# rrwick/Filtlong

Measured on AMD Instinct MI355X. Metric: Mbases/s scored+sorted, higher is better.
Workload: dtype f64; 1 GPU; 10,000,000 synthetic reads per GPU x gamma(k=4) mean 10 kbp, Phred-only, --target_bases 50008889515 (50% of bases); C2; reads_total=10000000, bases_total=100017779031, window_size=250, parallelism=1 GPU, device=AMD Radeon Graphics (gfx950:sramecc+:xnack-), gpus_visible=1, cut=select

## Files before the change

### filtlong_amd/csrc/fold_map.h

```cpp
#pragma once

#include <hip/hip_runtime.h>

namespace flx_fold {

constexpr int NO_MAP = -2147483647 - 1;

__device__ __forceinline__ int exponent_of(double v) {
    return (int)((__double_as_longlong(v) >> 52) & 0x7ff) - 1023;
}

struct Map2 {
    long long a0, a1;
};
__device__ __forceinline__ Map2 compose(const Map2 &a, const Map2 &b) {
    Map2 c;
    c.a0 = a.a0 + ((a.a0 & 1) ? b.a1 : b.a0);
    c.a1 = a.a1 + (((1 + a.a1) & 1) ? b.a1 : b.a0);
    return c;
}

__device__ __forceinline__ Map2 elem_map(double v, int e, bool &ok) {
    Map2 m;
    m.a0 = m.a1 = 0;
    const unsigned long long bits = (unsigned long long)__double_as_longlong(v);
    if ((bits << 1) == 0) return m;
    const int eb = (int)((bits >> 52) & 0x7ff);
    unsigned long long mx = bits & 0x000fffffffffffffull;
    int ex;
    if (eb == 0) ex = -1022;
    else { mx |= 1ull << 52; ex = eb - 1023; }
    const int sh = e - ex;
    if (sh < 0) { ok = false; return m; }
    if (sh == 0) { m.a0 = m.a1 = (long long)mx; return m; }
    if (sh >= 55) return m;
    const unsigned long long f = mx >> sh;
    const unsigned long long rem = mx & ((1ull << sh) - 1ull);
    const unsigned long long half = 1ull << (sh - 1);
    if (rem > half) m.a0 = m.a1 = (long long)(f + 1);
    else if (rem < half) m.a0 = m.a1 = (long long)f;
    else {
        m.a0 = (long long)(f + (f & 1));
        m.a1 = (long long)(f + ((f + 1) & 1));
    }
    return m;
}

__device__ __forceinline__ double readlane_f64(double v, int src) {
    const long long b = __double_as_longlong(v);
    const int lo = __builtin_amdgcn_readlane((int)(b & 0xffffffffll), src);
    const int hi = __builtin_amdgcn_readlane((int)(b >> 32), src);
    return __longlong_as_double(((long long)hi << 32) | (unsigned int)lo);
}

__device__ __forceinline__ bool normal_positive(double S) {
    const unsigned long long sb = (unsigned long long)__double_as_longlong(S);
    const int eb = (int)((sb >> 52) & 0x7ff);
    return (sb >> 63) == 0 && eb >= 1 && eb <= 2046;
}

}
```

### filtlong_amd/csrc/stats.hip

```cpp
#include <cmath>

#include "flx_internal.h"
#include "rank_internal.h"
#include "fold_map.h"

using namespace flx_fold;

namespace {

constexpr int CHUNK = 512;
constexpr int PER_LANE = CHUNK / 64;

struct Identity {
    double mean;
    __device__ __forceinline__ double operator()(double x) const { return x; }
};
struct SqDev {
    const double *mean;
    __device__ __forceinline__ double operator()(double x) const {
        const double d = x - *mean;
        return d * d;
    }
};

struct ChunkMeta {
    long long a0, a1;
    int e;
    int pad;
};

template <typename F>
__global__ void __launch_bounds__(256) k_chunk_sums(uint64_t n, const double *x, F f, double *chunk_sum, double *chunk_start,
                                                    unsigned char *chunk_clean, double *minmax) {
    const int lane = threadIdx.x & 63;
    const uint64_t chunk = (uint64_t)blockIdx.x * 4 + (threadIdx.x >> 6);
    const uint64_t base = chunk * CHUNK;
    if (base >= n) return;
    double acc = 0.0;
    bool clean = true;
    double lo = 100.0, hi = 0.0;
#pragma unroll
    for (int k = 0; k < PER_LANE; ++k) {
        const uint64_t i = base + (uint64_t)k * 64 + lane;
        if (i < n) {
            const double raw = x[i];
            const double v = f(raw);
            acc += v;
            clean = clean && (v >= 0.0) && (v < __longlong_as_double(0x7ff0000000000000ll));
            if (raw > hi) hi = raw;
            if (raw < lo) lo = raw;
        }
    }
    for (int o = 32; o > 0; o >>= 1) {
        acc += __shfl_xor(acc, o, 64);
        const double h2 = __shfl_xor(hi, o, 64), l2 = __shfl_xor(lo, o, 64);
        if (h2 > hi) hi = h2;
        if (l2 < lo) lo = l2;
    }
    const bool all_clean = __all(clean);
    if (lane == 0) {
        chunk_sum[chunk] = acc;
        chunk_start[chunk] = acc;
        chunk_clean[chunk] = all_clean ? 1 : 0;
        if (minmax) {
            minmax[2 * chunk] = lo;
            minmax[2 * chunk + 1] = hi;
        }
    }
}

__global__ void __launch_bounds__(256) k_minmax(uint64_t n_chunks, const double *minmax, double *out) {
    double lo = 100.0, hi = 0.0;
    for (uint64_t c = threadIdx.x; c < n_chunks; c += 256) {
        const double l = minmax[2 * c], h = minmax[2 * c + 1];
        if (l < lo) lo = l;
        if (h > hi) hi = h;
    }
    for (int o = 32; o > 0; o >>= 1) {
        const double l2 = __shfl_xor(lo, o, 64), h2 = __shfl_xor(hi, o, 64);
        if (l2 < lo) lo = l2;
        if (h2 > hi) hi = h2;
    }
    __shared__ double sl[4], sh[4];
    if ((threadIdx.x & 63) == 0) {
        sl[threadIdx.x >> 6] = lo;
        sh[threadIdx.x >> 6] = hi;
    }
    __syncthreads();
    if (threadIdx.x == 0) {
        for (int i = 1; i < 4; ++i) {
            if (sl[i] < lo) lo = sl[i];
            if (sh[i] > hi) hi = sh[i];
        }
        out[0] = lo;
        out[1] = hi;
    }
}

template <typename F>
__global__ void __launch_bounds__(256) k_chunk_maps(uint64_t n, const double *x, F f, const double *chunk_start,
                                                    const double *chunk_sum, const unsigned char *chunk_clean,
                                                    ChunkMeta *meta) {
    const int lane = threadIdx.x & 63;
    const uint64_t chunk = (uint64_t)blockIdx.x * 4 + (threadIdx.x >> 6);
    const uint64_t base = chunk * CHUNK;
    if (base >= n) return;
    const double p0 = chunk_start[chunk] * (1.0 - 1e-9);
    const double p1 = (chunk_start[chunk] + chunk_sum[chunk]) * (1.0 + 1e-9);
    int e = NO_MAP;
    if (chunk_clean[chunk] && p0 > 2.3e-308 && p1 < 1e300 && exponent_of(p0) == exponent_of(p1)) e = exponent_of(p0);
    Map2 m;
    m.a0 = m.a1 = 0;
    bool ok = true;
    if (e != NO_MAP) {
#pragma unroll
        for (int k = 0; k < PER_LANE; ++k) {
            const uint64_t i = base + (uint64_t)lane * PER_LANE + k;
            if (i < n) m = compose(m, elem_map(f(x[i]), e, ok));
        }
#pragma unroll
        for (int o = 1; o < 64; o <<= 1) {
            Map2 nb;
            nb.a0 = __shfl_down(m.a0, o, 64);
            nb.a1 = __shfl_down(m.a1, o, 64);
            if ((lane & (2 * o - 1)) == 0) m = compose(m, nb);
        }
        if (!__all(ok)) e = NO_MAP;
    }
    if (lane == 0) {
        ChunkMeta cm;
        cm.a0 = m.a0;
        cm.a1 = m.a1;
        cm.e = e;
        cm.pad = 0;
        meta[chunk] = cm;
    }
}

__global__ void __launch_bounds__(256) k_batch_maps(const ChunkMeta *meta, uint64_t n_chunks, ChunkMeta *batch) {
    const int lane = threadIdx.x & 63;
    const uint64_t b = (uint64_t)blockIdx.x * 4 + (threadIdx.x >> 6);
    const uint64_t c0 = b * 64;
    if (c0 >= n_chunks) return;
    ChunkMeta mine;
    mine.a0 = mine.a1 = 0;
    mine.e = NO_MAP;
    if (c0 + lane < n_chunks) mine = meta[c0 + lane];
    const int e0 = __builtin_amdgcn_readfirstlane(mine.e);
    const bool full = c0 + 64 <= n_chunks;
    Map2 m;
    m.a0 = mine.a0;
    m.a1 = mine.a1;
    const bool ok = full && e0 != NO_MAP && __all(mine.e == e0);
    if (ok) {
#pragma unroll
        for (int o = 1; o < 64; o <<= 1) {
            Map2 nb;
            nb.a0 = __shfl_down(m.a0, o, 64);
            nb.a1 = __shfl_down(m.a1, o, 64);
            if ((lane & (2 * o - 1)) == 0) m = compose(m, nb);
        }
    }
    if (lane == 0) {
        ChunkMeta out;
        out.a0 = m.a0;
        out.a1 = m.a1;
        out.e = ok ? e0 : NO_MAP;
        out.pad = 0;
        batch[b] = out;
    }
}

__device__ __forceinline__ bool apply_map(double &S, int e, long long a0, long long a1) {
    const unsigned long long sb = (unsigned long long)__double_as_longlong(S);
    const int se = (int)((sb >> 52) & 0x7ff) - 1023;
    if (se != e || (sb >> 63) != 0 || a0 < 0 || a1 < 0) return false;
    const unsigned long long m = (sb & 0x000fffffffffffffull) | (1ull << 52);
    const unsigned long long m2 = m + (unsigned long long)((m & 1) ? a1 : a0);
    if (m2 > (1ull << 53)) return false;
    if (m2 == (1ull << 53)) S = __longlong_as_double((long long)(((unsigned long long)(e + 1 + 1023)) << 52));
    else S = __longlong_as_double((long long)((((unsigned long long)(e + 1023)) << 52) | (m2 & 0x000fffffffffffffull)));
    return true;
}

__device__ __forceinline__ Map2 wave_scan_maps(Map2 m, int lane) {
#pragma unroll
    for (int o = 1; o < 64; o <<= 1) {
        Map2 prev;
        prev.a0 = __shfl_up(m.a0, o, 64);
        prev.a1 = __shfl_up(m.a1, o, 64);
        if (lane >= o) m = compose(prev, m);
    }
    return m;
}

__device__ __forceinline__ int wave_apply_prefix(double &S, int e, Map2 m, bool usable, int start, int lane) {
    const bool good = usable && m.a0 >= 0 && m.a1 >= 0;
    const unsigned long long bad = __ballot(lane >= start && !good);
    const int first_bad = bad ? (int)__ffsll((long long)bad) - 1 : 64;
    if (lane < start || lane >= first_bad) m.a0 = m.a1 = 0;
    const Map2 P = wave_scan_maps(m, lane);
    const unsigned long long sb = (unsigned long long)__double_as_longlong(S);
    const unsigned long long ms = (sb & 0x000fffffffffffffull) | (1ull << 52);
    const unsigned long long m2 = ms + (unsigned long long)((ms & 1) ? P.a1 : P.a0);
    const bool inside = m2 <= (1ull << 53);
    const unsigned long long out = __ballot(lane >= start && lane < first_bad && !inside);
    const int f = out ? (int)__ffsll((long long)out) - 1 : first_bad;
    if (f > start) {
        const unsigned int lo = (unsigned int)__builtin_amdgcn_readlane((int)(m2 & 0xffffffffull), f - 1);
        const unsigned int hi = (unsigned int)__builtin_amdgcn_readlane((int)(m2 >> 32), f - 1);
        const unsigned long long r = ((unsigned long long)hi << 32) | lo;
        if (r == (1ull << 53)) S = __longlong_as_double((long long)(((unsigned long long)(e + 1 + 1023)) << 52));
        else S = __longlong_as_double((long long)((((unsigned long long)(e + 1023)) << 52) | (r & 0x000fffffffffffffull)));
    }
    return f;
}

template <typename F>
__global__ void __launch_bounds__(64) k_walk(uint64_t n, const double *x, F f, const ChunkMeta *meta, const ChunkMeta *batch,
                                             uint64_t n_chunks, flx_stats_dev *out, int second) {
    const int lane = threadIdx.x;
    double S = 0.0;
    unsigned long long n_serial = 0;
    const uint64_t n_batches = (n_chunks + 63) / 64;
    for (uint64_t bb = 0; bb < n_batches && S == S; bb += 64) {
        ChunkMeta bm;
        bm.a0 = bm.a1 = 0;
        bm.e = NO_MAP;
        if (bb + lane < n_batches) bm = batch[bb + lane];
        const int bcnt = (int)((n_batches - bb) < 64 ? (n_batches - bb) : 64);
        int bs = 0;
        while (bs < bcnt && S == S) {
            int fb = bs;
            if (normal_positive(S)) {
                const int e = exponent_of(S);
                Map2 m;
                m.a0 = bm.a0;
                m.a1 = bm.a1;
                fb = wave_apply_prefix(S, e, m, lane < bcnt && bm.e == e, bs, lane);
            }
            if (fb >= bcnt) break;
            const uint64_t cb = (bb + fb) * 64;
            ChunkMeta mine;
            mine.a0 = mine.a1 = 0;
            mine.e = NO_MAP;
            if (cb + lane < n_chunks) mine = meta[cb + lane];
            const int cnt = (int)((n_chunks - cb) < 64 ? (n_chunks - cb) : 64);
            int cs = 0;
            while (cs < cnt && S == S) {
                int fc = cs;
                if (normal_positive(S)) {
                    const int e = exponent_of(S);
                    Map2 m;
                    m.a0 = mine.a0;
                    m.a1 = mine.a1;
                    fc = wave_apply_prefix(S, e, m, lane < cnt && mine.e == e, cs, lane);
                }
                if (fc >= cnt) break;
                ++n_serial;
                const uint64_t chunk = cb + fc;
                const uint64_t base = chunk * CHUNK;
                double v[PER_LANE];
#pragma unroll
                for (int j = 0; j < PER_LANE; ++j) {
                    const uint64_t i = base + (uint64_t)lane * PER_LANE + j;
                    v[j] = i < n ? f(x[i]) : 0.0;
                }
                const int m_el = (int)((n - base) < CHUNK ? (n - base) : CHUNK);
                const int n_lanes = (m_el + PER_LANE - 1) / PER_LANE;
                int ls = 0, opened = 0;
                while (ls < n_lanes && S == S) {
                    int fl = ls;
                    if (chunk != 0 && opened < 4 && normal_positive(S)) {
                        const int e = exponent_of(S);
                        Map2 m;
                        m.a0 = m.a1 = 0;
                        bool ok = true;
#pragma unroll
                        for (int j = 0; j < PER_LANE; ++j) {
                            if (lane * PER_LANE + j < m_el) {
                                const double xv = v[j];
                                if (xv >= 0.0 && xv < __longlong_as_double(0x7ff0000000000000ll)) m = compose(m, elem_map(xv, e, ok));
                                else ok = false;
                            }
                        }
                        fl = wave_apply_prefix(S, e, m, ok && lane < n_lanes, ls, lane);
                    }
                    if (fl >= n_lanes) break;
#pragma unroll
                    for (int j = 0; j < PER_LANE; ++j)
                        if (fl * PER_LANE + j < m_el) S += readlane_f64(v[j], fl);
                    ++opened;
                    ls = fl + 1;
                }
                cs = fc + 1;
            }
            bs = fb + 1;
        }
    }
    if (lane == 0) {
        const double nn = (double)n;
        if (!second) {
            out->sum = S;
            out->mean = S / nn;
        } else {
            out->sq_sum = S;
            out->stdev = sqrt(S / nn);
        }
        out->serial_chunks[second] = n_serial;
    }
}

template <typename F>
int exact_fold(flx_ctx *ctx, uint64_t n, const double *x, F f, char *ws, flx_stats_dev *d_out, int second) {
    double *d_minmax_out = second ? nullptr : &d_out->min;
    const uint64_t n_chunks = (n + CHUNK - 1) / CHUNK;
    double *chunk_sum = (double *)ws;
    double *chunk_start = chunk_sum + n_chunks;
    double *minmax = chunk_start + n_chunks;
    ChunkMeta *meta = (ChunkMeta *)(minmax + 2 * n_chunks);
    const uint64_t n_batches = (n_chunks + 63) / 64;
    ChunkMeta *batch = meta + n_chunks;
    unsigned char *clean = (unsigned char *)(batch + n_batches);
    char *scan_ws = (char *)(((uintptr_t)(clean + n_chunks) + 255) & ~(uintptr_t)255);
    hipStream_t st = ctx->stream;
    const unsigned nb = (unsigned)((n_chunks + 3) / 4);
    hipLaunchKernelGGL(k_chunk_sums<F>, dim3(nb), dim3(256), 0, st, n, x, f, chunk_sum, chunk_start, clean,
                       d_minmax_out ? minmax : (double *)nullptr);
    if (d_minmax_out) hipLaunchKernelGGL(k_minmax, dim3(1), dim3(256), 0, st, n_chunks, minmax, d_minmax_out);
    FLX_CHECK(flx_exclusive_scan_f64_approx(ctx, n_chunks, chunk_start, scan_ws));
    hipLaunchKernelGGL(k_chunk_maps<F>, dim3(nb), dim3(256), 0, st, n, x, f, chunk_start, chunk_sum, clean, meta);
    hipLaunchKernelGGL(k_batch_maps, dim3((unsigned)((n_batches + 3) / 4)), dim3(256), 0, st, meta, n_chunks, batch);
    hipLaunchKernelGGL(k_walk<F>, dim3(1), dim3(64), 0, st, n, x, f, meta, batch, n_chunks, d_out, second);
    FLX_HIP(ctx, hipGetLastError());
    return FLX_OK;
}

}

size_t flx_exact_stats_workspace(uint64_t n) {
    const uint64_t n_chunks = (n + CHUNK - 1) / CHUNK;
    return n_chunks * (8 + 8 + 16 + sizeof(ChunkMeta) + 1) + (n_chunks / 64 + 2) * sizeof(ChunkMeta) + 512 + (n_chunks / 2048 + 4096) * 8 * 2 + 4096;
}

int flx_exact_stats_async(flx_ctx *ctx, uint64_t n, const double *d_mean_q, void *ws, flx_stats_dev *d_out) {
    flx_time_scope t(ctx, "flx_rank_stats");
    FLX_CHECK(exact_fold(ctx, n, d_mean_q, Identity{0.0}, (char *)ws, d_out, 0));
    FLX_CHECK(exact_fold(ctx, n, d_mean_q, SqDev{&d_out->mean}, (char *)ws, d_out, 1));
    return FLX_OK;
}

bool flx_stats_finish(const flx_stats_dev &h, uint64_t n, flx_stats *out) {
    memset(out, 0, sizeof *out);
    out->sum = h.sum;
    out->min = h.min;
    out->max = h.max;
    out->sq_sum = h.sq_sum;
    {
        volatile double s = out->sum, nn = (double)n;
        out->mean = s / nn;
    }
    {
        volatile double ss = out->sq_sum, nn = (double)n;
        out->stdev = sqrt(ss / nn);
    }
    out->serial_chunks = h.serial_chunks[0] + h.serial_chunks[1];
    return memcmp(&out->mean, &h.mean, 8) == 0 && memcmp(&out->stdev, &h.stdev, 8) == 0;
}

int flx_exact_stats(flx_ctx *ctx, uint64_t n, const double *d_mean_q, flx_stats *out) {
    memset(out, 0, sizeof *out);
    if (n == 0) {
        volatile double z = 0.0;
        out->min = 100.0; out->max = 0.0; out->sum = 0.0; out->mean = z / z; out->sq_sum = 0.0; out->stdev = sqrt(z / z);
        return FLX_OK;
    }
    void *scr;
    FLX_CHECK(flx_scratch(ctx, 256 + flx_exact_stats_workspace(n), &scr));
    flx_stats_dev *d_out = (flx_stats_dev *)scr;
    char *ws = (char *)scr + 256;
    FLX_CHECK(flx_exact_stats_async(ctx, n, d_mean_q, ws, d_out));
    flx_stats_dev h;
    FLX_HIP(ctx, hipMemcpyAsync(&h, d_out, sizeof h, hipMemcpyDeviceToHost, ctx->stream));
    FLX_HIP(ctx, hipStreamSynchronize(ctx->stream));
    flx_stats_finish(h, n, out);
    if (memcmp(&out->mean, &h.mean, 8) != 0) {
        FLX_HIP(ctx, hipMemcpyAsync(&d_out->mean, &out->mean, 8, hipMemcpyHostToDevice, ctx->stream));
        FLX_CHECK(exact_fold(ctx, n, d_mean_q, SqDev{&d_out->mean}, ws, d_out, 1));
        FLX_HIP(ctx, hipMemcpyAsync(&h, d_out, sizeof h, hipMemcpyDeviceToHost, ctx->stream));
        FLX_HIP(ctx, hipStreamSynchronize(ctx->stream));
        h.mean = out->mean;
        flx_stats_finish(h, n, out);
    }
    return FLX_OK;
}
```

Before: 3.572 million Mbases/s.

## Pre-stage per-lane maps for exponent-crossing chunks and use DPP wave scan

Chunks whose approximate prefix range spans exactly one exponent boundary now have per-lane rounding maps precomputed in parallel for both candidate exponents, stored in up to 24 staged slots. The serial single-wave walk loads these into shared memory and applies them directly instead of recomputing element maps when it reaches such chunks. The wave prefix scan of maps is also switched from shfl_up to DPP row operations. This aims to cut the serial walk's per-chunk latency, at the cost of extra map computation, atomics and workspace in the parallel kernel.

```diff
diff --git a/filtlong_amd/csrc/fold_map.h b/filtlong_amd/csrc/fold_map.h
--- a/filtlong_amd/csrc/fold_map.h
+++ b/filtlong_amd/csrc/fold_map.h
@@ -1,6 +1,22 @@
 #pragma once
 
+#if defined(__HIPCC__)
 #include <hip/hip_runtime.h>
+#else
+#include <cstring>
+#define __device__
+#define __forceinline__ inline
+inline long long __double_as_longlong(double v) {
+    long long b;
+    memcpy(&b, &v, sizeof b);
+    return b;
+}
+inline double __longlong_as_double(long long b) {
+    double v;
+    memcpy(&v, &b, sizeof v);
+    return v;
+}
+#endif
 
 namespace flx_fold {
 
@@ -46,12 +62,14 @@
     return m;
 }
 
+#if defined(__HIPCC__)
 __device__ __forceinline__ double readlane_f64(double v, int src) {
     const long long b = __double_as_longlong(v);
     const int lo = __builtin_amdgcn_readlane((int)(b & 0xffffffffll), src);
     const int hi = __builtin_amdgcn_readlane((int)(b >> 32), src);
     return __longlong_as_double(((long long)hi << 32) | (unsigned int)lo);
 }
+#endif
 
 __device__ __forceinline__ bool normal_positive(double S) {
     const unsigned long long sb = (unsigned long long)__double_as_longlong(S);
diff --git a/filtlong_amd/csrc/stats.hip b/filtlong_amd/csrc/stats.hip
--- a/filtlong_amd/csrc/stats.hip
+++ b/filtlong_amd/csrc/stats.hip
@@ -3,6 +3,7 @@
 #include "flx_internal.h"
 #include "rank_internal.h"
 #include "fold_map.h"
+#include "stats_walk.h"
 
 using namespace flx_fold;
 
@@ -31,9 +32,10 @@
 
 template <typename F>
 __global__ void __launch_bounds__(256) k_chunk_sums(uint64_t n, const double *x, F f, double *chunk_sum, double *chunk_start,
-                                                    unsigned char *chunk_clean, double *minmax) {
+                                                    unsigned char *chunk_clean, double *minmax, unsigned int *n_staged) {
     const int lane = threadIdx.x & 63;
     const uint64_t chunk = (uint64_t)blockIdx.x * 4 + (threadIdx.x >> 6);
+    if (blockIdx.x == 0 && threadIdx.x == 0) *n_staged = 0;
     const uint64_t base = chunk * CHUNK;
     if (base >= n) return;
     double acc = 0.0;
@@ -97,10 +99,14 @@
     }
 }
 
+struct StagedMaps {
+    Map2 m[STAGE_SLOTS][2][64];
+};
+
 template <typename F>
 __global__ void __launch_bounds__(256) k_chunk_maps(uint64_t n, const double *x, F f, const double *chunk_start,
                                                     const double *chunk_sum, const unsigned char *chunk_clean,
-                                                    ChunkMeta *meta) {
+                                                    ChunkMeta *meta, StagedMaps *staged, unsigned int *n_staged) {
     const int lane = threadIdx.x & 63;
     const uint64_t chunk = (uint64_t)blockIdx.x * 4 + (threadIdx.x >> 6);
     const uint64_t base = chunk * CHUNK;
@@ -108,7 +114,34 @@
     const double p0 = chunk_start[chunk] * (1.0 - 1e-9);
     const double p1 = (chunk_start[chunk] + chunk_sum[chunk]) * (1.0 + 1e-9);
     int e = NO_MAP;
-    if (chunk_clean[chunk] && p0 > 2.3e-308 && p1 < 1e300 && exponent_of(p0) == exponent_of(p1)) e = exponent_of(p0);
+    int pad = 0;
+    {
+        int e0;
+        const int guess = guess_chunk(chunk_clean[chunk] != 0, p0, p1, chunk == 0, &e0);
+        if (guess == GUESS_MAP) e = e0;
+        if (guess == GUESS_STAGE) {
+            Map2 m0, m1;
+            m0.a0 = m0.a1 = m1.a0 = m1.a1 = 0;
+            bool ok0 = true, ok1 = true;
+#pragma unroll
+            for (int k = 0; k < PER_LANE; ++k) {
+                const uint64_t i = base + (uint64_t)lane * PER_LANE + k;
+                if (i < n) {
+                    const double v = f(x[i]);
+                    m0 = compose(m0, elem_map(v, e0, ok0));
+                    m1 = compose(m1, elem_map(v, e0 + 1, ok1));
+                }
+            }
+            unsigned int slot = 0;
+            if (lane == 0) slot = atomicAdd(n_staged, 1u);
+            slot = (unsigned int)__builtin_amdgcn_readfirstlane((int)slot);
+            if (slot < (unsigned int)STAGE_SLOTS) {
+                staged->m[slot][0][lane] = staged_lane_map(m0, ok0);
+                staged->m[slot][1][lane] = staged_lane_map(m1, ok1);
+                pad = staged_tag((int)slot, e0);
+            }
+        }
+    }
     Map2 m;
     m.a0 = m.a1 = 0;
     bool ok = true;
@@ -132,7 +165,7 @@
         cm.a0 = m.a0;
         cm.a1 = m.a1;
         cm.e = e;
-        cm.pad = 0;
+        cm.pad = pad;
         meta[chunk] = cm;
     }
 }
@@ -183,14 +216,26 @@
     return true;
 }
 
-__device__ __forceinline__ Map2 wave_scan_maps(Map2 m, int lane) {
-#pragma unroll
-    for (int o = 1; o < 64; o <<= 1) {
-        Map2 prev;
-        prev.a0 = __shfl_up(m.a0, o, 64);
-        prev.a1 = __shfl_up(m.a1, o, 64);
-        if (lane >= o) m = compose(prev, m);
-    }
+template <int CTRL, int ROW_MASK>
+__device__ __forceinline__ long long dpp_or_zero(long long v) {
+    const int lo = __builtin_amdgcn_update_dpp(0, (int)(v & 0xffffffffll), CTRL, ROW_MASK, 0xf, false);
+    const int hi = __builtin_amdgcn_update_dpp(0, (int)(v >> 32), CTRL, ROW_MASK, 0xf, false);
+    return ((long long)hi << 32) | (unsigned int)lo;
+}
+template <int CTRL, int ROW_MASK>
+__device__ __forceinline__ Map2 scan_step(const Map2 &m) {
+    Map2 prev;
+    prev.a0 = dpp_or_zero<CTRL, ROW_MASK>(m.a0);
+    prev.a1 = dpp_or_zero<CTRL, ROW_MASK>(m.a1);
+    return compose(prev, m);
+}
+__device__ __forceinline__ Map2 wave_scan_maps(Map2 m) {
+    m = scan_step<0x111, 0xf>(m);
+    m = scan_step<0x112, 0xf>(m);
+    m = scan_step<0x114, 0xf>(m);
+    m = scan_step<0x118, 0xf>(m);
+    m = scan_step<0x142, 0xa>(m);
+    m = scan_step<0x143, 0xc>(m);
     return m;
 }
 
@@ -199,27 +244,30 @@
     const unsigned long long bad = __ballot(lane >= start && !good);
     const int first_bad = bad ? (int)__ffsll((long long)bad) - 1 : 64;
     if (lane < start || lane >= first_bad) m.a0 = m.a1 = 0;
-    const Map2 P = wave_scan_maps(m, lane);
-    const unsigned long long sb = (unsigned long long)__double_as_longlong(S);
-    const unsigned long long ms = (sb & 0x000fffffffffffffull) | (1ull << 52);
-    const unsigned long long m2 = ms + (unsigned long long)((ms & 1) ? P.a1 : P.a0);
-    const bool inside = m2 <= (1ull << 53);
+    const Map2 P = wave_scan_maps(m);
+    const unsigned long long m2 = mantissa_after(S, P);
+    const bool inside = mantissa_inside(m2);
     const unsigned long long out = __ballot(lane >= start && lane < first_bad && !inside);
     const int f = out ? (int)__ffsll((long long)out) - 1 : first_bad;
     if (f > start) {
         const unsigned int lo = (unsigned int)__builtin_amdgcn_readlane((int)(m2 & 0xffffffffull), f - 1);
         const unsigned int hi = (unsigned int)__builtin_amdgcn_readlane((int)(m2 >> 32), f - 1);
-        const unsigned long long r = ((unsigned long long)hi << 32) | lo;
-        if (r == (1ull << 53)) S = __longlong_as_double((long long)(((unsigned long long)(e + 1 + 1023)) << 52));
-        else S = __longlong_as_double((long long)((((unsigned long long)(e + 1023)) << 52) | (r & 0x000fffffffffffffull)));
+        S = sum_from_mantissa(e, ((unsigned long long)hi << 32) | lo);
     }
     return f;
 }
 
 template <typename F>
 __global__ void __launch_bounds__(64) k_walk(uint64_t n, const double *x, F f, const ChunkMeta *meta, const ChunkMeta *batch,
-                                             uint64_t n_chunks, flx_stats_dev *out, int second) {
+                                             uint64_t n_chunks, const StagedMaps *staged, flx_stats_dev *out, int second) {
     const int lane = threadIdx.x;
+    __shared__ StagedMaps s_staged;
+#pragma unroll
+    for (int s = 0; s < STAGE_SLOTS; ++s) {
+        s_staged.m[s][0][lane] = staged->m[s][0][lane];
+        s_staged.m[s][1][lane] = staged->m[s][1][lane];
+    }
+    __builtin_amdgcn_wave_barrier();
     double S = 0.0;
     unsigned long long n_serial = 0;
     const uint64_t n_batches = (n_chunks + 63) / 64;
@@ -244,6 +292,7 @@
             ChunkMeta mine;
             mine.a0 = mine.a1 = 0;
             mine.e = NO_MAP;
+            mine.pad = 0;
             if (cb + lane < n_chunks) mine = meta[cb + lane];
             const int cnt = (int)((n_chunks - cb) < 64 ? (n_chunks - cb) : 64);
             int cs = 0;
@@ -260,15 +309,36 @@
                 ++n_serial;
                 const uint64_t chunk = cb + fc;
                 const uint64_t base = chunk * CHUNK;
-                double v[PER_LANE];
-#pragma unroll
-                for (int j = 0; j < PER_LANE; ++j) {
-                    const uint64_t i = base + (uint64_t)lane * PER_LANE + j;
-                    v[j] = i < n ? f(x[i]) : 0.0;
-                }
                 const int m_el = (int)((n - base) < CHUNK ? (n - base) : CHUNK);
                 const int n_lanes = (m_el + PER_LANE - 1) / PER_LANE;
                 int ls = 0, opened = 0;
+                const int pad = __builtin_amdgcn_readlane(mine.pad, fc);
+                if (pad != 0) {
+                    const int slot = staged_slot(pad), e0 = staged_e0(pad);
+                    for (int t = 0; t < 2 && ls < n_lanes && normal_positive(S); ++t) {
+                        const int set = staged_set_for(S, e0);
+                        if (set < 0) break;
+                        const Map2 m = s_staged.m[slot][set][lane];
+                        const int fl = wave_apply_prefix(S, e0 + set, m, lane < n_lanes, ls, lane);
+                        ls = fl;
+                        if (fl >= n_lanes || t == 1) break;
+                        const uint64_t i = base + (uint64_t)fl * PER_LANE + lane;
+                        const double sv = (lane < PER_LANE && i < n) ? f(x[i]) : 0.0;
+#pragma unroll
+                        for (int j = 0; j < PER_LANE; ++j)
+                            if (fl * PER_LANE + j < m_el) S += readlane_f64(sv, j);
+                        ++opened;
+                        ls = fl + 1;
+                    }
+                }
+                double v[PER_LANE] = {};
+                if (ls < n_lanes) {
+#pragma unroll
+                    for (int j = 0; j < PER_LANE; ++j) {
+                        const uint64_t i = base + (uint64_t)lane * PER_LANE + j;
+                        v[j] = i < n ? f(x[i]) : 0.0;
+                    }
+                }
                 while (ls < n_lanes && S == S) {
                     int fl = ls;
                     if (chunk != 0 && opened < 4 && normal_positive(S)) {
@@ -310,6 +380,8 @@
         out->serial_chunks[second] = n_serial;
     }
 }
+
+size_t scan_workspace_bytes(uint64_t n_chunks) { return (n_chunks / 2048 + 4096) * 8 * 2; }
 
 template <typename F>
 int exact_fold(flx_ctx *ctx, uint64_t n, const double *x, F f, char *ws, flx_stats_dev *d_out, int second) {
@@ -323,15 +395,18 @@
     ChunkMeta *batch = meta + n_chunks;
     unsigned char *clean = (unsigned char *)(batch + n_batches);
     char *scan_ws = (char *)(((uintptr_t)(clean + n_chunks) + 255) & ~(uintptr_t)255);
+    StagedMaps *staged = (StagedMaps *)(((uintptr_t)(scan_ws + scan_workspace_bytes(n_chunks)) + 255) & ~(uintptr_t)255);
+    unsigned int *n_staged = (unsigned int *)(staged + 1);
     hipStream_t st = ctx->stream;
     const unsigned nb = (unsigned)((n_chunks + 3) / 4);
     hipLaunchKernelGGL(k_chunk_sums<F>, dim3(nb), dim3(256), 0, st, n, x, f, chunk_sum, chunk_start, clean,
-                       d_minmax_out ? minmax : (double *)nullptr);
+                       d_minmax_out ? minmax : (double *)nullptr, n_staged);
     if (d_minmax_out) hipLaunchKernelGGL(k_minmax, dim3(1), dim3(256), 0, st, n_chunks, minmax, d_minmax_out);
     FLX_CHECK(flx_exclusive_scan_f64_approx(ctx, n_chunks, chunk_start, scan_ws));
-    hipLaunchKernelGGL(k_chunk_maps<F>, dim3(nb), dim3(256), 0, st, n, x, f, chunk_start, chunk_sum, clean, meta);
+    hipLaunchKernelGGL(k_chunk_maps<F>, dim3(nb), dim3(256), 0, st, n, x, f, chunk_start, chunk_sum, clean, meta, staged,
+                       n_staged);
     hipLaunchKernelGGL(k_batch_maps, dim3((unsigned)((n_batches + 3) / 4)), dim3(256), 0, st, meta, n_chunks, batch);
-    hipLaunchKernelGGL(k_walk<F>, dim3(1), dim3(64), 0, st, n, x, f, meta, batch, n_chunks, d_out, second);
+    hipLaunchKernelGGL(k_walk<F>, dim3(1), dim3(64), 0, st, n, x, f, meta, batch, n_chunks, staged, d_out, second);
     FLX_HIP(ctx, hipGetLastError());
     return FLX_OK;
 }
@@ -340,7 +415,8 @@
 
 size_t flx_exact_stats_workspace(uint64_t n) {
     const uint64_t n_chunks = (n + CHUNK - 1) / CHUNK;
-    return n_chunks * (8 + 8 + 16 + sizeof(ChunkMeta) + 1) + (n_chunks / 64 + 2) * sizeof(ChunkMeta) + 512 + (n_chunks / 2048 + 4096) * 8 * 2 + 4096;
+    return n_chunks * (8 + 8 + 16 + sizeof(ChunkMeta) + 1) + (n_chunks / 64 + 2) * sizeof(ChunkMeta) + 512 + scan_workspace_bytes(n_chunks) + 256 +
+           sizeof(StagedMaps) + 256 + 4096;
 }
 
 int flx_exact_stats_async(flx_ctx *ctx, uint64_t n, const double *d_mean_q, void *ws, flx_stats_dev *d_out) {
diff --git a/filtlong_amd/csrc/stats_walk.h b/filtlong_amd/csrc/stats_walk.h
--- /dev/null
+++ b/filtlong_amd/csrc/stats_walk.h
@@ -0,0 +1,44 @@
+#pragma once
+
+#include "fold_map.h"
+
+namespace flx_fold {
+
+constexpr int STAGE_SLOTS = 24;
+
+__device__ __forceinline__ int staged_tag(int slot, int e0) { return (slot + 1) | ((e0 + 1023) << 8); }
+__device__ __forceinline__ int staged_slot(int tag) { return (tag & 0xff) - 1; }
+__device__ __forceinline__ int staged_e0(int tag) { return (tag >> 8) - 1023; }
+
+enum { GUESS_NONE = 0, GUESS_MAP = 1, GUESS_STAGE = 2 };
+__device__ __forceinline__ int guess_chunk(bool clean, double p0, double p1, bool first_chunk, int *e) {
+    *e = NO_MAP;
+    if (!clean || !(p0 > 2.3e-308) || !(p1 < 1e300)) return GUESS_NONE;
+    const int e0 = exponent_of(p0), e1 = exponent_of(p1);
+    if (e1 == e0) { *e = e0; return GUESS_MAP; }
+    if (e1 == e0 + 1 && !first_chunk) { *e = e0; return GUESS_STAGE; }
+    return GUESS_NONE;
+}
+
+__device__ __forceinline__ Map2 staged_lane_map(Map2 m, bool ok) {
+    if (!ok) m.a0 = m.a1 = -1;
+    return m;
+}
+
+__device__ __forceinline__ int staged_set_for(double S, int e0) {
+    const int e = exponent_of(S);
+    return e == e0 ? 0 : (e == e0 + 1 ? 1 : -1);
+}
+
+__device__ __forceinline__ unsigned long long mantissa_after(double S, const Map2 &P) {
+    const unsigned long long sb = (unsigned long long)__double_as_longlong(S);
+    const unsigned long long ms = (sb & 0x000fffffffffffffull) | (1ull << 52);
+    return ms + (unsigned long long)((ms & 1) ? P.a1 : P.a0);
+}
+__device__ __forceinline__ bool mantissa_inside(unsigned long long m2) { return m2 <= (1ull << 53); }
+__device__ __forceinline__ double sum_from_mantissa(int e, unsigned long long m2) {
+    if (m2 == (1ull << 53)) return __longlong_as_double((long long)(((unsigned long long)(e + 1 + 1023)) << 52));
+    return __longlong_as_double((long long)((((unsigned long long)(e + 1023)) << 52) | (m2 & 0x000fffffffffffffull)));
+}
+
+}
```

Measured after the change: 3.585 million Mbases/s (median of 6 runs). No clear change (+0.4%).
